# ehsan886/DBA_mod

Hardware: AMD Instinct MI355X
Metric: FL rounds/sec + backdoor ASR & main-task acc, ResNet-18 CIFAR-10 100 clients (higher is better)
Workload: dtype fp32

## Files before the change

### csrc/kernels/xaux.hip

```cpp
#include "common.hpp"
#include "xmfma.hpp"
#include <algorithm>

namespace {

__device__ __forceinline__ void xsplit_w_body(const float* __restrict__ w, long long sstride, long long per,
                                              const int* __restrict__ amax, int ld, uint16_t* __restrict__ out,
                                              int sl, long long e0, long long e1, long long step) {
  const int sb = hexp(amax_read(amax, ld, sl));
  const float mb = __uint_as_float((uint32_t)(sb + 127) << 23);
  const float* __restrict__ src = w + (long long)sl * sstride;
  uint16_t* __restrict__ oh = out + (long long)sl * 2 * per;
  uint16_t* __restrict__ ol = oh + per;
  for (long long e = e0 + threadIdx.x * 4LL; e < e1; e += step) {
    float v[4];
#pragma unroll
    for (int i = 0; i < 4; ++i) v[i] = e + i < per ? src[e + i] : 0.f;
    uint2 sp[2];
    split4h(v[0], v[1], v[2], v[3], mb, sp);
    const uint16_t* h = (const uint16_t*)&sp[0];
    const uint16_t* l = (const uint16_t*)&sp[1];
#pragma unroll
    for (int i = 0; i < 4; ++i)
      if (e + i < per) { oh[e + i] = h[i]; ol[e + i] = l[i]; }
  }
}
__global__ __launch_bounds__(256) void xsplit_w_kernel(const float* __restrict__ w, long long sstride, long long per,
                                                       const int* __restrict__ amax, int ld,
                                                       uint16_t* __restrict__ out) {
  xsplit_w_body(w, sstride, per, amax, ld, out, blockIdx.y, blockIdx.x * 1024LL, per, (long long)gridDim.x * 1024);
}
struct XSDesc {
  long long w, sstride, per, amax, ld, out, boff;
};
constexpr int kXSBatch = 24, kXSChunk = 4096;
struct XSBatch {
  XSDesc d[kXSBatch];
  int n;
};
__global__ __launch_bounds__(256) void xsplit_w_batch_kernel(const XSBatch b) {
  int i = 0;
  while (i + 1 < b.n && (long long)blockIdx.x >= b.d[i + 1].boff) ++i;
  const XSDesc& d = b.d[i];
  const long long e0 = ((long long)blockIdx.x - d.boff) * kXSChunk;
  const long long e1 = e0 + kXSChunk < d.per ? e0 + kXSChunk : d.per;
  xsplit_w_body((const float*)d.w, d.sstride, d.per, (const int*)d.amax, (int)d.ld, (uint16_t*)d.out, blockIdx.y, e0,
                e1, 1024);
}

constexpr int kAmaxSegs = 64, kAmaxChunk = 4096;
struct AmaxSegs {
  long long off[kAmaxSegs];
  int len[kAmaxSegs];
  int start[kAmaxSegs + 1];
  int n;
};
__global__ __launch_bounds__(256) void amax_segments_kernel(const float* __restrict__ base, long long gstride,
                                                            const AmaxSegs segs, int ld, int* __restrict__ out) {
  const int c = blockIdx.x, g = blockIdx.y;
  int sg = 0;
  while (sg + 1 < segs.n && segs.start[sg + 1] <= c) ++sg;
  const float* __restrict__ p = base + (long long)g * gstride + segs.off[sg];
  const int n = segs.len[sg], e0 = (c - segs.start[sg]) * kAmaxChunk;
  const bool v4 = ((segs.off[sg] | gstride) & 3) == 0 && ((uintptr_t)base & 15) == 0;
  float m = 0.f;
  float4 v[4];
#pragma unroll
  for (int k = 0; k < 4; ++k) {
    const int e = e0 + (k * 256 + threadIdx.x) * 4;
    if (v4 && e + 3 < n) {
      v[k] = *(const float4*)(p + e);
    } else {
      v[k].x = e < n ? p[e] : 0.f;
      v[k].y = e + 1 < n ? p[e + 1] : 0.f;
      v[k].z = e + 2 < n ? p[e + 2] : 0.f;
      v[k].w = e + 3 < n ? p[e + 3] : 0.f;
    }
  }
#pragma unroll
  for (int k = 0; k < 4; ++k) m = fmaxf(m, fmaxf(fmaxf(fabsf(v[k].x), fabsf(v[k].y)), fmaxf(fabsf(v[k].z), fabsf(v[k].w))));
  amax_fold(out + (long long)sg * kAmaxSub * ld, ld, g, m);
}

__global__ __launch_bounds__(256) void amax_kernel(const float* __restrict__ x, long long gstride, long long n_per_g,
                                                   const int* __restrict__ nvalid, long long per_item, int vec,
                                                   int* __restrict__ out, int ld) {
  const int g = blockIdx.y;
  const long long n = nvalid ? (long long)nvalid[g] * per_item : n_per_g;
  const float* __restrict__ p = x + (long long)g * gstride;
  float m = 0.f;
  if (vec) {
    const long long n4 = n >> 2;
    for (long long e = blockIdx.x * 256LL + threadIdx.x; e < n4; e += (long long)gridDim.x * 256) {
      const float4 v = ((const float4*)p)[e];
      m = fmaxf(m, fmaxf(fmaxf(fabsf(v.x), fabsf(v.y)), fmaxf(fabsf(v.z), fabsf(v.w))));
    }
    for (long long e = n4 * 4 + blockIdx.x * 256LL + threadIdx.x; e < n; e += (long long)gridDim.x * 256)
      m = fmaxf(m, fabsf(p[e]));
  } else {
    for (long long e = blockIdx.x * 256LL + threadIdx.x; e < n; e += (long long)gridDim.x * 256) m = fmaxf(m, fabsf(p[e]));
  }
  amax_fold(out, ld, g, m);
}

}

DBA_EXPORT int dba_xsplit_w(const float* w, long long sstride, long long per, int slots, const int* amax, int ld,
                            uint16_t* out, void* stream) {
  const dim3 grid((unsigned)std::max(1LL, std::min(1024LL, (per + 1023) / 1024)), slots);
  hipLaunchKernelGGL(xsplit_w_kernel, grid, dim3(256), 0, (hipStream_t)stream, w, sstride, per, amax, ld, out);
  DBA_LAUNCH_CHECK();
}


DBA_EXPORT int dba_xsplit_w_batch(const void* desc, int n, int slots, void* stream) {
  const XSDesc* ds = (const XSDesc*)desc;
  for (int i0 = 0; i0 < n; i0 += kXSBatch) {
    XSBatch b{};
    b.n = std::min(kXSBatch, n - i0);
    long long nb = 0;
    for (int i = 0; i < b.n; ++i) {
      b.d[i] = ds[i0 + i];
      b.d[i].boff = nb;
      nb += (b.d[i].per + kXSChunk - 1) / kXSChunk;
    }
    hipLaunchKernelGGL(xsplit_w_batch_kernel, dim3((unsigned)nb, slots), dim3(256), 0, (hipStream_t)stream, b);
    const int rc = (int)hipGetLastError();
    if (rc != 0) return rc;
  }
  return 0;
}


DBA_EXPORT int dba_amax_segments(const float* base, long long gstride, const long long* segs, int n, int G, int* out,
                                 int ld, void* stream) {
  if (n > kAmaxSegs || n < 1) return -105;
  AmaxSegs a{};
  a.n = n;
  for (int i = 0; i < n; ++i) {
    a.off[i] = segs[2 * i];
    a.len[i] = (int)segs[2 * i + 1];
    a.start[i + 1] = a.start[i] + std::max(1, ceil_div(a.len[i], kAmaxChunk));
  }
  const dim3 grid((unsigned)a.start[n], G);
  hipLaunchKernelGGL(amax_segments_kernel, grid, dim3(256), 0, (hipStream_t)stream, base, gstride, a, ld, out);
  DBA_LAUNCH_CHECK();
}


DBA_EXPORT int dba_amax(const float* x, long long gstride, long long n_per_g, const int* nvalid, long long per_item,
                        int G, int* out, int ld, void* stream) {
  hipStream_t st = (hipStream_t)stream;
  const int vec = aligned16(x) && gstride % 4 == 0;
  const long long per = nvalid ? per_item * (n_per_g / std::max(1LL, per_item)) : n_per_g;
  const dim3 grid((unsigned)std::max(1LL, std::min(256LL, (per + 4095) / 4096)), G);
  hipLaunchKernelGGL(amax_kernel, grid, dim3(256), 0, st, x, gstride, n_per_g, nvalid, per_item, vec, out, ld);
  DBA_LAUNCH_CHECK();
}
```

### csrc/kernels/xconv.hpp

```cpp
#pragma once
#include "common.hpp"
#include "bnfuse.hpp"
#include "xmfma.hpp"
#include <algorithm>
#include <type_traits>
#include <utility>
#include <cstdlib>

namespace xg {
struct SplitPolicy {
  int target = 128, min_k = 8, max_s = 8, kslab_max = 2;
  int dgrad_ks = 1;
};
SplitPolicy& split_policy();
int bnx_tile_go(const ::BnFuse& f, const float* src, float* dst, long long gstride, const int* nvalid, int G, int N,
                int HW, const float* pool, float pool_scale, const float* ws, int S, long long zstride,
                const float* accum, hipStream_t st);
}
using xg::SplitPolicy;
using xg::split_policy;
using xg::bnx_tile_go;

namespace {

struct XClass {
  int nI, nJ;
  int bh, bw;
  int oh, ow;
  int Hq, Wq;
  long long boff;
};

struct XArgs {
  const float* src; long long src_gstride;
  const float* w; long long w_sstride;
  const int* wsel;
  const float* bias; long long b_sstride;
  const float* res;
  float* out; long long out_gstride;
  const int* nvalid;
  int N, Hs, Ws, Cs, Ncol, Ho, Wo;
  int sp, os, dsg, relu;
  int splitk, tiles_n;
  int kslab;
  long long zstride;
  const int* amax_src;
  const int* amax_w;
  int* amax_out;
  int amax_src_ld, amax_w_ld, amax_out_ld;
  const uint16_t* wp;
  long long wp_sstride;
  float* sk_ws; long long sk_gstride;
  int* sk_cnt;
  BnFuse bf;
  const float* lz_coef;
  int lz_relu;
  const float* sc_src; long long sc_gstride;
  int sc_H, sc_W, sc_C;
  const uint16_t* sc_wp; long long sc_wp_sstride;
  const int* sc_amax_src; int sc_amax_src_ld;
  const int* sc_amax_w; int sc_amax_w_ld;
  const float* sc_bias; long long sc_b_sstride;
  XClass cls[4];
};

typedef __attribute__((ext_vector_type(4))) unsigned int u32x4v;

constexpr int kSkMax = 8;
template <int BM, int BN>
__device__ __forceinline__ bool sk_combine(const XArgs& a, float* Ct, const long long* orow, int g, int zc, int kz,
                                           int n0, int* flag) {
  constexpr int C4 = BN / 4, IT = BM * C4 / 256;
  static_assert(BM * C4 % 256 == 0, "whole float4 passes");
  const int tid = threadIdx.x, S = a.splitk;
  const float* base = a.sk_ws + (long long)g * a.sk_gstride;
  int off[IT];
#pragma unroll
  for (int it = 0; it < IT; ++it) {
    const int e = tid + it * 256, row = e / C4, cc = (e - row * C4) * 4, n = n0 + cc;
    const long long o = orow[row];
    off[it] = (o < 0 || n >= a.Ncol) ? kOOB : (int)((o + n) * 4);
  }
  {
    const __amdgpu_buffer_rsrc_t rs = rsrc(base + (long long)kz * a.zstride, a.sk_gstride * 4);
#pragma unroll
    for (int it = 0; it < IT; ++it) {
      const int e = tid + it * 256, row = e / C4, cc = (e - row * C4) * 4;
      const float4 v = *(const float4*)&Ct[row * BN + cc];
      if (off[it] != kOOB)
        __builtin_amdgcn_raw_buffer_store_b128(__builtin_bit_cast(u32x4v, v), rs, off[it], 0, 16);
    }
  }
  asm volatile("s_waitcnt vmcnt(0)" ::: "memory");
  __syncthreads();
  if (tid == 0) {
    int* cnt = a.sk_cnt + ((long long)g * gridDim.x + blockIdx.x) * (gridDim.z / S) + zc;
    const int t = __hip_atomic_fetch_add(cnt, 1, __ATOMIC_RELAXED, __HIP_MEMORY_SCOPE_AGENT);
    const int last = t == S - 1;
    if (last) __hip_atomic_store(cnt, 0, __ATOMIC_RELAXED, __HIP_MEMORY_SCOPE_AGENT);
    *flag = last;
  }
  __syncthreads();
  if (!*flag) return false;
  __builtin_amdgcn_fence(__ATOMIC_ACQUIRE, "wavefront");
  float4 w[kSkMax][IT];
#pragma unroll
  for (int z = 0; z < kSkMax; ++z) {
    if (z < S && z != kz) {
      const __amdgpu_buffer_rsrc_t rz = rsrc(base + (long long)z * a.zstride, a.sk_gstride * 4);
#pragma unroll
      for (int it = 0; it < IT; ++it)
        w[z][it] = __builtin_bit_cast(float4, __builtin_amdgcn_raw_buffer_load_b128(rz, off[it], 0, 16));
    }
  }
#pragma unroll
  for (int it = 0; it < IT; ++it) {
    const int e = tid + it * 256, row = e / C4, cc = (e - row * C4) * 4;
    float4* cp = (float4*)&Ct[row * BN + cc];
    const float4 own = *cp;
    float4 v = kz == 0 ? own : w[0][it];
#pragma unroll
    for (int z = 1; z < kSkMax; ++z) {
      if (z < S) {
        const float4 u = z == kz ? own : w[z][it];
        v.x += u.x; v.y += u.y; v.z += u.z; v.w += u.w;
      }
    }
    if (off[it] != kOOB) *cp = v;
  }
  __syncthreads();
  return true;
}

#ifndef XCONV_MINB
// ... 437 lines not shown
```

### csrc/kernels/xconv_fwd.hip

```cpp
#include "xhalo.hpp"

namespace xg {
SplitPolicy& split_policy() {
  static SplitPolicy p;
  return p;
}
}

namespace {

template <int W, int IMGS, int BN, int WM, int WN, bool PRE>
__global__ __launch_bounds__(256) void ximg_kernel(const XArgs a) {
  constexpr int P = 2, NT = 256;
  constexpr int PW = W + 2, PI = PW * PW, PP = IMGS * PI;
  constexpr int CC = 32, CH = CC / 8, Q4 = CC / 4;
  constexpr int PATCH = PP * CH;
  constexpr int BM = IMGS * W * W;
  constexpr int TM = BM / WM, TN = BN / WN, MI = TM / 32, NJ = TN / 32;
  static_assert(WM * WN == NT / 64 && MI >= 1 && NJ >= 1 && BM == 128, "tiling");
  constexpr int RPT = NT / 8;
  static_assert(BN % RPT == 0, "weight rows");
  constexpr int RB = BN / RPT, BPL = BN * 4;
  __shared__ __attribute__((aligned(16))) uint4 patch[P * PATCH];
  __shared__ __attribute__((aligned(16))) uint4 bring[2 * P * BPL];
// ... 98 lines not shown
#pragma unroll
      for (int i = 0; i < MI; ++i) {
        const int pp = apix[i] + toff;
        const int o = pp * CH + (ch ^ ((arow[i] + ti) & 3));
#pragma unroll
        for (int p = 0; p < P; ++p) af[p][i] = patch[p * PATCH + o];
      }
#pragma unroll
      for (int j = 0; j < NJ; ++j) {
        const int n = wn * TN + j * 32 + fr;
        const int o = n * 4 + (ch ^ ((n >> 2) & 3));
#pragma unroll
        for (int p = 0; p < P; ++p) bfr[p][j] = L[p * BPL + o];
      }
      mma_half<MI, NJ, P, true, RB, decltype(KK)::value>(af, bfr, acc, [&](int q) __attribute__((always_inline)) {
        lput_q(buf ^ 1, stn, q);
        gq(t + 3, stn, q);
      });
    });
  };
  auto step = [&](int t, int buf, int stn) __attribute__((always_inline)) {
    const int c = t / 9;
    mma(t, buf, stn);
    __syncthreads();
    if (t - 9 * c == 8 && c + 1 < NC) {
#pragma unroll
      for (int u = 0; u < NE; ++u) ppiece(u, hs.ma);
      if (c + 2 < NC) pload(c + 2);
      __syncthreads();
    }
  };

  hs.init(amax_read(a.amax_src, a.amax_src_ld, g), amax_read(a.amax_w, a.amax_w_ld, slot));
#pragma unroll
  for (int q = 0; q < RB; ++q) {
    gq(0, 0, q);
    gq(1, 1, q);
  }
  pload(0);
#pragma unroll
  for (int u = 0; u < NE; ++u) ppiece(u, hs.ma);
  if (NC > 1) pload(1);
#pragma unroll
  for (int q = 0; q < RB; ++q) {
    lput_q(0, 0, q);
    gq(2, 0, q);
  }
  __syncthreads();
  int t = 0;
  for (; t + 1 < NK; t += 2) {
    step(t, 0, 1);
    step(t + 1, 1, 0);
  }
  if (t < NK) step(t, 0, 1);
  hs.finish(acc);

  float* out = a.out + (long long)g * a.out_gstride;
  const float* bias = a.bias ? a.bias + (long long)slot * a.b_sstride : nullptr;
  const float* res = a.res ? a.res + (long long)g * a.out_gstride : nullptr;
  float vmax = 0.f;
#pragma unroll
  for (int j = 0; j < NJ; ++j) {
    const int n = n0 + wn * TN + j * 32 + fr;
    if (n >= a.Ncol) continue;
    const float bv = bias ? bias[n] : 0.f;
#pragma unroll
    for (int i = 0; i < MI; ++i)
#pragma unroll
      for (int r = 0; r < 16; ++r) {
        const int m = wm * TM + i * 32 + (r & 3) + 8 * (r >> 2) + 4 * hf;
        if (img0 + m / (W * W) >= nv) continue;
        const long long o = (long long)(img0 * W * W + m) * a.Ncol + n;
        float v = acc[i][j][r];
        if (bias) v += bv;
        if (res) v += res[o];
        if (a.relu) v = fmaxf(v, 0.f);
        vmax = fmaxf(vmax, fabsf(v));
        out[o] = v;
      }
  }
  if (a.amax_out) amax_fold(a.amax_out, a.amax_out_ld, g, vmax);
}

template <int W, int IMGS, int BN, int WM, int WN>
int ximg_go(const XArgs& a, int G, hipStream_t st) {
  XArgs b = a;
  b.tiles_n = ceil_div(a.Ncol, BN);
  const dim3 grid((unsigned)(ceil_div(a.N, IMGS) * b.tiles_n), G, 1);
  if (a.wp) hipLaunchKernelGGL((ximg_kernel<W, IMGS, BN, WM, WN, true>), grid, dim3(256), 0, st, b);
  else hipLaunchKernelGGL((ximg_kernel<W, IMGS, BN, WM, WN, false>), grid, dim3(256), 0, st, b);
  DBA_LAUNCH_CHECK();
}
int& ximg_on() {
  static int on = 1;
  return on;
}
int ximg_try(const XArgs& a, int G, int KH, int KW, hipStream_t st) {
  const XClass& c = a.cls[0];
  if (!ximg_on() || KH != 3 || KW != 3 || a.sp != 1 || a.os != 1 || a.dsg != 1 || a.splitk != 1 || c.nI != 3 ||
      c.nJ != 3 || c.bh != -1 || c.bw != -1)
    return -100;
  if (a.Hs != a.Ho || a.Ws != a.Wo || a.Ho != a.Wo || a.Cs % 32 != 0 || a.Ncol % 32 != 0) return -100;
  if (a.bf.mode || a.lz_coef) return -100;
  if (!aligned16(a.src) || a.src_gstride % 4 || !aligned16(a.w) || a.w_sstride % 4) return -100;
  if (a.wp && (((uintptr_t)a.wp & 15) || a.wp_sstride % 8)) return -100;
  if (a.sc_src) return -100;
  if (a.Wo == 8) return a.Ncol >= 128 ? ximg_go<8, 2, 128, 2, 2>(a, G, st) : ximg_go<8, 2, 64, 2, 2>(a, G, st);
  if (a.Wo == 4) return a.Ncol >= 128 ? ximg_go<4, 8, 128, 2, 2>(a, G, st) : ximg_go<4, 8, 64, 2, 2>(a, G, st);
  return -100;
}

}

DBA_EXPORT int dba_xsplit_policy(int target, int min_k, int max_s, int kslab_max, int dgrad_ks) {
  SplitPolicy& p = split_policy();
  if (dgrad_ks >= 0) p.dgrad_ks = dgrad_ks;
  if (target > 0) p.target = target;
  if (min_k > 0) p.min_k = min_k;
  if (max_s > 0) p.max_s = std::min(max_s, kSkMax);
  if (kslab_max > 0) p.kslab_max = kslab_max;
  return 0;
}

DBA_EXPORT int dba_ximg_set(int on) {
  const int prev = ximg_on();
  if (on >= 0) ximg_on() = on;
  return prev;
}


DBA_EXPORT long long dba_xconv_ws_floats(int G, int N, int Ho, int Wo, int Cin, int Cout, int KH, int KW) {
  const long long M = (long long)N * Ho * Wo;
  const int s = xsplitk(M, G, Cout, KH * KW * Cin);
  return s > 1 ? (long long)s * G * M * Cout : 0;
}


DBA_EXPORT long long dba_xconv_sk_ints(int G, int N, int Ho, int Wo, int Cin, int Cout, int KH, int KW) {
  const long long M = (long long)N * Ho * Wo;
  const int s = xsplitk(M, G, Cout, KH * KW * Cin);
  const long long n = s > 1 ? xconv_sk_count(M, Cout, G, 1, s) : 0;
  return (n > 0 && sk_ok((const int*)1, n, M, Cout, G, 1, s)) ? n : 0;
}


DBA_EXPORT int dba_xconv_fwd(const float* x, long long x_gstride, const float* w, long long w_sstride,
                             const int* wsel, const float* bias, long long b_sstride, const float* res, float* out,
                             long long out_gstride, const int* nvalid, int G, int N, int H, int W, int Cin, int Ho,
                             int Wo, int Cout, int KH, int KW, int stride, int pad, int relu, const int* amax_x,
                             int amax_x_ld, const int* amax_w, int amax_w_ld, int* amax_out, int amax_out_ld,
                             const uint16_t* wp, long long wp_sstride, float* ws, long long ws_floats, int* sk_cnt,
                             long long sk_cnt_n, const void* bnf, const float* lz_coef, int lz_relu,
                             void* stream) {
  hipStream_t st = (hipStream_t)stream;
  if ((long long)N * H * W * Cin >= (1LL << 29)) return -103;
  const long long M = (long long)N * Ho * Wo;
  const int K = KH * KW * Cin;
  const int vec = (Cin % 4 == 0 && aligned16(x) && aligned16(w) && x_gstride % 4 == 0 && w_sstride % 4 == 0) ? 4 : 1;
  XArgs a{};
  a.src = x; a.src_gstride = x_gstride; a.w = w; a.w_sstride = w_sstride; a.wsel = wsel;
  a.bias = bias; a.b_sstride = b_sstride; a.res = res; a.out = out; a.out_gstride = out_gstride;
  a.nvalid = nvalid; a.N = N; a.Hs = H; a.Ws = W; a.Cs = Cin; a.Ncol = Cout; a.Ho = Ho; a.Wo = Wo;
  a.sp = stride; a.os = 1; a.dsg = 1; a.relu = relu; a.splitk = 1;
  a.amax_src = amax_x; a.amax_w = amax_w; a.amax_out = amax_out;
  a.amax_src_ld = amax_x_ld; a.amax_w_ld = amax_w_ld; a.amax_out_ld = amax_out_ld;
  a.wp = wp; a.wp_sstride = wp_sstride;
  a.cls[0] = XClass{KH, KW, -pad, -pad, 0, 0, Ho, Wo, 0};
  if (!amax_x || !amax_w) return -109;
  if (bnf) {
    a.bf = *(const BnFuse*)bnf;
    if (a.bf.mode != 1 || bias || res || relu || (Cout & 3) || a.bf.C != Cout) return -108;
  }
  if (lz_coef) {
    if (wp || vec < 4 || Cin > 512) return -108;
    a.lz_coef = lz_coef; a.lz_relu = lz_relu;
  }
  auto fin = [&](int rc) { return (rc == 0 && a.bf.mode) ? bnx_finalize_go(a.bf, nvalid, G, N, Ho * Wo, st) : rc; };
  if (stride == 1) {
    int rc = ximg_try(a, G, KH, KW, st);
    if (rc == -100) rc = xhalo_try(a, G, KH, KW, st);
    if (rc != -100) return fin(rc);
  }
  const int s = xsplitk(M, G, Cout, K);
  const bool ws_ok = s > 1 && ws != nullptr && ws_floats >= (long long)s * G * M * Cout;
  if (s > 1 && !(ws_ok && sk_ok(sk_cnt, sk_cnt_n, M, Cout, G, 1, s))) {
    XArgs b = a;
    b.kslab = s;
    const int rc = xconv_ks(b, M, G, vec, st);
    if (rc != -100) return fin(rc);
  }
  if (ws_ok && sk_ok(sk_cnt, sk_cnt_n, M, Cout, G, 1, s)) {
    XArgs b = a;
    b.splitk = s;
    b.zstride = (long long)G * M * Cout;
    b.sk_ws = ws; b.sk_gstride = M * Cout; b.sk_cnt = sk_cnt;
    return fin(xconv_dispatch(b, M, G, 1, vec, st));
  }
  if (ws_ok) {
    XArgs b = a;
    b.splitk = s;
    b.out = ws;
    b.out_gstride = M * Cout;
    b.zstride = (long long)G * M * Cout;
    const int rc = xconv_dispatch(b, M, G, 1, vec, st);
    if (rc != 0) return rc;
    if (a.bf.mode)
      return bnx_tile_go(a.bf, nullptr, out, out_gstride, nvalid, G, N, Ho * Wo, nullptr, 0.f, ws, s, b.zstride,
                         nullptr, st);
    const long long per = M * Cout;
    const dim3 grid((unsigned)std::max(1LL, std::min(1024LL, (per + 255) / 256)), G);
    hipLaunchKernelGGL(xsplitk_reduce_kernel, grid, dim3(256), 0, st, (const float*)ws, s, b.zstride, per, nvalid, N,
                       Ho * Wo, Cout, bias, b_sstride, wsel, res, relu, out, amax_out, amax_out_ld);
    DBA_LAUNCH_CHECK();
  }
  return fin(xconv_dispatch(a, M, G, 1, vec, st));
}


DBA_EXPORT int dba_xdown_fwd(const float* a_, long long a_gstride, const float* w2, long long w2_sstride,
                             const uint16_t* w2p, long long w2p_sstride, const int* wsel, const float* b2,
                             long long b_sstride, const float* x2, long long x2_gstride, const uint16_t* wscp,
                             long long wscp_sstride, const float* bsc, long long bsc_sstride, float* out,
                             long long out_gstride, const int* nvalid, int G, int N, int Ho, int Wo, int C, int H2,
                             int W2, int C2, const int* amax_a, int amax_a_ld, const int* amax_w2, int amax_w2_ld,
                             const int* amax_x2, int amax_x2_ld, const int* amax_wsc, int amax_wsc_ld, int* amax_out,
                             int amax_out_ld, void* stream) {
  if (!amax_a || !amax_w2 || !amax_x2 || !amax_wsc || !w2p || !wscp) return -109;
  if ((H2 - 1) / 2 + 1 != Ho || (W2 - 1) / 2 + 1 != Wo || (long long)N * H2 * W2 * C2 >= (1LL << 29) ||
      (long long)N * Ho * Wo * C >= (1LL << 29))
    return -103;
  XArgs a{};
  a.src = a_; a.src_gstride = a_gstride; a.w = w2; a.w_sstride = w2_sstride; a.wsel = wsel;
  a.bias = b2; a.b_sstride = b_sstride; a.res = nullptr; a.out = out; a.out_gstride = out_gstride;
  a.nvalid = nvalid; a.N = N; a.Hs = Ho; a.Ws = Wo; a.Cs = C; a.Ncol = C; a.Ho = Ho; a.Wo = Wo;
  a.sp = 1; a.os = 1; a.dsg = 1; a.relu = 1; a.splitk = 1;
  a.amax_src = amax_a; a.amax_w = amax_w2; a.amax_out = amax_out;
  a.amax_src_ld = amax_a_ld; a.amax_w_ld = amax_w2_ld; a.amax_out_ld = amax_out_ld;
  a.wp = w2p; a.wp_sstride = w2p_sstride;
  a.sc_src = x2; a.sc_gstride = x2_gstride; a.sc_H = H2; a.sc_W = W2; a.sc_C = C2;
  a.sc_wp = wscp; a.sc_wp_sstride = wscp_sstride;
  a.sc_amax_src = amax_x2; a.sc_amax_src_ld = amax_x2_ld; a.sc_amax_w = amax_wsc; a.sc_amax_w_ld = amax_wsc_ld;
  a.sc_bias = bsc; a.sc_b_sstride = bsc_sstride;
  a.cls[0] = XClass{3, 3, -1, -1, 0, 0, Ho, Wo, 0};
  return xhalo_try(a, G, 3, 3, (hipStream_t)stream);
}
```

### dba_mod_amd/ops/hip.py

```python
from __future__ import annotations

import contextlib
import ctypes
import os
from typing import Optional, Sequence, Tuple

import torch

from . import bnstate as bs
from . import build

Tensor = torch.Tensor
_F32 = torch.float32

if not os.path.exists(build.kernels_path()):
    raise ImportError(f"HIP kernel library missing: {build.kernels_path()} — run "
                      f"`python -m dba_mod_amd.ops.build` (or __graft_entry__.build())")
_L = ctypes.CDLL(build.kernels_path())

_P = ctypes.c_void_p
_I = ctypes.c_int
_LL = ctypes.c_longlong
_F = ctypes.c_float
_U = ctypes.c_uint
_D = ctypes.c_double

_SIGS = {
    "dba_gather_images": [_P, _P, _P, _P, _P, _P, _I, _P, _P, _I, _P, _I, _I, _I, _I, _I, _P],
    "dba_gather_rows": [_P, _P, _P, _P, _P, _I, _P, _P, _I, _P, _I, _P, _I, _I, _I, _P],
    "dba_xcolsum": [_P, _LL, _I, _P, _I, _I, _I, _P, _LL, _P, _P],
    "dba_xcolsum_part_doubles": [_I, _I, _I, _I],
    "dba_amax_segments": [_P, _LL, _P, _I, _I, _P, _I, _P],
    "dba_bn_fold": [_P, _LL, _P, _P, _P, _P, _P, _LL, _F, _P, _P, _I, _I, _I, _I, _P, _I, _P],
    "dba_relu_mask_bwd": [_P, _P, _P, _LL, _I, _P],
    "dba_maxpool": [_P, _P, _P, _LL, _I, _I, _I, _I, _I, _I, _I, _I, _I, _P],
    "dba_maxpool_bwd": [_P, _P, _P, _LL, _I, _I, _I, _I, _I, _I, _I, _I, _I, _P],
    "dba_avgpool": [_P, _P, _LL, _I, _I, _I, _P],
    "dba_avgpool_bwd": [_P, _P, _LL, _I, _I, _I, _P],
    "dba_dropout": [_P, _P, _I, _P, _U, _F, _LL, _I, _P],
    "dba_softmax_xent": [_P, _P, _I, _I, _I, _I, _P, _P, _P, _P, _LL, _P, _I, _P, _I, _P, _P, _P],
    "dba_softmax_xent_part_doubles": [_I, _I],
    "dba_xent_r5_set": [_I],
    "dba_head_train": [_P, _LL, _I, _I, _I, _I, _P, _LL, _P, _LL, _I, _P, _P, _P, _P, _P, _P, _LL, _P, _LL, _P, _P,
                       _P, _P, _LL, _P, _I, _I, _P],
    "dba_head_part_doubles": [_I, _I],
    "dba_sgd_step": [_P, _LL, _P, _P, _P, _P, _P, _F, _F, _P, _I, _I, _P],
    "dba_scale_from_base": [_P, _P, _F, _P, _LL, _P],
    "dba_add_noise_scaled": [_P, _P, _LL, _F, _F, _U, _I, _I, _P],
    "dba_delta_sum": [_P, _LL, _I, _P, _LL, _P, _P],
    "dba_sqdist_blocks": [_LL],
    "dba_gram_chunks": [_I],
    "dba_sq_dists": [_P, _LL, _P, _I, _LL, _P, _P, _P],
    "dba_weighted_sum": [_P, _LL, _P, _I, _P, _LL, _I, _P],
    "dba_weighted_sum_fixed": [_P, _LL, _P, _I, _P, _LL, _D, _P],
    "dba_gram": [_P, _LL, _I, _I, _P, _P, _P],
    "dba_dist_loss_grad": [_P, _LL, _P, _LL, _P, _LL, _I, _P, _P, _F, _P, _P, _P],
    "dba_ximg_set": [_I],
    "dba_xwgrad_halo_set": [_I],
    "dba_xconv_ws_floats": [_I] * 8,
    "dba_xconv_fwd": [_P, _LL, _P, _LL, _P, _P, _LL, _P, _P, _LL, _P] + [_I] * 13 + [_P, _I] * 3 + [_P, _LL] * 2
    + [_P, _LL, _P, _P, _I, _P],
    "dba_xconv_sk_ints": [_I] * 8,
    "dba_xconv_dgrad": [_P, _LL, _P, _LL, _P, _P, _P, _LL, _P] + [_I] * 12 + [_P, _I] * 2 + [_P, _LL] * 3 + [_P, _P],
    "dba_xsplit_w": [_P, _LL, _LL, _I, _P, _I, _P, _P],
    "dba_amax": [_P, _LL, _LL, _P, _LL, _I, _P, _I, _P],
    "dba_xtranspose": [_P, _I, _I, _LL, _P, _P],
    "dba_xwgrad_ws_floats": [_I] * 8 + [_P],
    "dba_xwgrad_stem_ws_floats": [_I] * 6,
    "dba_xsplit_policy": [_I] * 5,
    "dba_xsplit_w_batch": [_P, _I, _I, _P],
    "dba_bn_fold_batch": [_P, _I, _I, _F, _P],
    "dba_xwgrad": [_P, _LL, _P, _LL, _P, _LL, _P] + [_I] * 12 + [_P, _I] * 2 + [_P, _LL, _I] + [_P, _I, _P],
    "dba_bnx_rows": [_P, _P, _P, _LL, _P, _I, _I, _I, _P, _F, _P],
    "dba_bnx_apply": [_P, _P, _P, _P, _P, _I, _I, _P, _LL, _P, _I, _I, _I, _I, _P, _I, _P],
    "dba_bnfuse_size": [],
    "dba_xwgrad_stem": [_P, _LL, _P, _P, _P, _LL, _P, _P, _I, _I, _I, _I, _P],
    "dba_bnx_dy": [_P, _P, _P, _P, _LL, _P, _I, _I, _I, _I, _P, _I, _P],
    "dba_xwgrad_reduce_batch": [_P, _I, _I, _LL, _P],
    "dba_xblock_fwd": [_P, _LL, _P, _LL, _P, _P, _P, _LL, _P, _P, _LL, _P] + [_I] * 6
    + [_P, _I, _P, _P, _I, _P, _I, _P],
    "dba_xblock_stem_fwd": [_P, _LL, _P, _LL, _P, _P, _LL, _P, _LL, _P, _P, _LL, _P, _P, _LL, _P] + [_I] * 6
    + [_P, _P, _P, _I, _P, _I, _P],
    "dba_mlp_train": [_P, _I, _I, _I, _I, _I, _P, _LL, _P, _P, _I, _P, _I, _I, _I, _I, _P, _P, _P, _P, _I, _I,
                      _P, _LL, _I, _P, _F, _F, _P, _P],
    "dba_xdown_fwd": [_P, _LL, _P, _LL, _P, _LL, _P, _P, _LL, _P, _LL, _P, _LL, _P, _LL, _P, _LL, _P] + [_I] * 8
    + [_P, _I] * 5 + [_P],
    "dba_xstem_fwd": [_P, _LL, _P, _LL, _P, _P, _LL, _P, _P, _LL, _P] + [_I] * 13 + [_P, _I, _P, _P],
}
for _name, _args in _SIGS.items():
    _fn = getattr(_L, _name)
    _fn.argtypes = _args
    _fn.restype = ctypes.c_int
_L.dba_xconv_ws_floats.restype = ctypes.c_longlong
_L.dba_xconv_sk_ints.restype = ctypes.c_longlong
_L.dba_xwgrad_ws_floats.restype = ctypes.c_longlong
_L.dba_xwgrad_stem_ws_floats.restype = ctypes.c_longlong
_L.dba_xcolsum_part_doubles.restype = ctypes.c_longlong
_L.dba_softmax_xent_part_doubles.restype = ctypes.c_longlong
_L.dba_head_part_doubles.restype = ctypes.c_longlong


class _BnFuse(ctypes.Structure):
    _fields_ = [("mode", _I), ("C", _I), ("ngrp", _I),
                ("rec0", _P),
                ("coef_a", _P), ("gamma_a", _P), ("beta_a", _P), ("rm_a", _P), ("rv_a", _P),
                ("p_gstride", _LL), ("momentum", _F), ("eps", _F), ("relu", _I),
                ("amax_a", _P), ("amax_ld", _I),
                ("ya", _P), ("yb", _P), ("y_gstride", _LL),
                ("coef_b", _P), ("gamma_b", _P), ("amax_b", _P),
                ("dgamma_a", _P), ("dbeta_a", _P), ("dgamma_b", _P), ("dbeta_b", _P), ("gr_gstride", _LL),
                ("mask_out", _P), ("mask_lazy", _I)]


assert ctypes.sizeof(_BnFuse) == int(_L.dba_bnfuse_size()), "BnFuse layout mismatch (rebuild the kernels)"


NOT_HANDLED = -100
F16_PAIR = 16


def _call(name: str, *args) -> int:
    rc = getattr(_L, name)(*args)
    if rc != 0 and rc != NOT_HANDLED:
        raise RuntimeError(f"{name}: HIP error {rc}")
    return rc


def _ptr(t: Optional[Tensor]):
    return None if t is None else t.data_ptr()


def _stream():
    return torch.cuda.current_stream().cuda_stream


def _i32(t: Optional[Tensor]) -> Optional[Tensor]:
    if t is None:
        return None
    return t if (t.dtype == torch.int32 and t.is_contiguous()) else t.to(torch.int32).contiguous()


def _inner_contig(t: Tensor) -> bool:
    exp = 1
    for d in range(t.dim() - 1, 0, -1):
        if t.shape[d] != 1 and t.stride(d) != exp:
            return False
        exp *= t.shape[d]
    return True


def _rowview(t: Tensor) -> Tuple[Tensor, int]:
    if not _inner_contig(t):
        t = t.contiguous()
# ... 121 lines not shown
        flat = torch.zeros(slots + counters, dtype=torch.int32, device=device)
        self.buf = flat[:slots].view(n, AMAX_SUB, self.ld)
        self.cnt, self.cnt_next = flat[slots:], 0

    def counters(self, n: int, device):
        if n <= 0 or device != self.cnt.device or self.cnt_next + n > self.cnt.numel():
            return None
        self.cnt_next += n
        return self.cnt[self.cnt_next - n:self.cnt_next]

    def take(self, G: int, device):
        if G != self.G or self.next >= self.buf.shape[0] or device != self.buf.device:
            return None
        self.next += 1
        return self.buf[self.next - 1]


_ARENA: list = []


@contextlib.contextmanager
def amax_arena(G: int, device, n: int = 256, counters: int = 0):
    _ARENA.append(_AmaxArena(G, device, n, counters))
    try:
        yield
    finally:
        _ARENA.pop()


def amax_slots(n: int, G: int, device):
    return torch.zeros(n, AMAX_SUB, _amax_ld(G), dtype=torch.int32, device=device)


def _amax_new(G: int, device):
    a = _ARENA[-1].take(G, device) if _ARENA else None
    return a if a is not None else torch.zeros(AMAX_SUB, _amax_ld(G), dtype=torch.int32, device=device)


def _sk_counters(n: int, device):
    if n <= 0 or not _ARENA:
        return None
    return _ARENA[-1].counters(n, device)


def _aptr(a):
    return (None, 0) if a is None else (a.data_ptr(), a.shape[-1])


def _amax(t, gstride, n_per_g, nvalid=None, per_item=0):
    G = t.shape[0]
    out = _amax_new(G, t.device)
    _call("dba_amax", t.data_ptr(), gstride, n_per_g, _ptr(_i32(nvalid)), per_item, G, out.data_ptr(), out.shape[1],
          _stream())
    return out


def _amax_out(t):
    if t.dtype != _F32:
        return None
    a = _amax_new(t.shape[0], t.device)
    t._dba_amax = a
    return a


def weight_amax(flat, segments):
    G, n = flat.shape[0], len(segments)
    ar = _ARENA[-1] if _ARENA else None
    if ar is not None and ar.G == G and ar.buf.device == flat.device and ar.next + n <= ar.buf.shape[0]:
        buf, ar.next = ar.buf[ar.next:ar.next + n], ar.next + n
    else:
        buf = torch.zeros(n, AMAX_SUB, _amax_ld(G), dtype=torch.int32, device=flat.device)
    slots, base = list(buf), buf.data_ptr()
    d = torch.tensor(segments, dtype=torch.int64)
    _call("dba_amax_segments", flat.data_ptr(), flat.stride(0), d.data_ptr(), len(segments), G, base,
          slots[0].shape[1], _stream())
    return slots


def split_weights(w, sstride: int, per: int, amax):
    slots = w.shape[0]
    out = torch.empty(slots, 2, per, dtype=torch.int16, device=w.device)
    _call("dba_xsplit_w", w.data_ptr(), sstride, per, slots, amax.data_ptr(), amax.shape[1], out.data_ptr(), _stream())
    w._dba_planes = out
    return out


def split_weights_batch(items) -> None:
    if not items:
        return
    slots = items[0][0].shape[0]
    desc, outs = [], []
    for w, sstride, per, amax in items:
        assert w.shape[0] == slots and w.dtype == torch.float32
        out = torch.empty(slots, 2, per, dtype=torch.int16, device=w.device)
        desc.append([w.data_ptr(), sstride, per, amax.data_ptr(), amax.shape[1], out.data_ptr(), 0])
        outs.append(out)
    d = torch.tensor(desc, dtype=torch.int64)
    _call("dba_xsplit_w_batch", d.data_ptr(), len(items), slots, _stream())
    for (w, *_), out in zip(items, outs):
        w._dba_planes = out


def _wplanes(w):
    p = getattr(w, "_dba_planes", None)
    return (None, 0) if p is None else (p.data_ptr(), p.stride(0))


def _amax_w(w, gstride, n):
    a = getattr(w, "_dba_amax", None)
    if a is None:
        a = _amax(w, gstride, n)
        w._dba_amax = a
    return a


def _amax_act(t, nvalid):
    a = getattr(t, "_dba_amax", None)
    if a is not None:
        return a
    per_item = t[0, 0].numel()
    a = _amax(t, t.stride(0), t.shape[1] * per_item, nvalid, per_item)
    t._dba_amax = a
    return a


_EVAL_STEM_MFMA = os.environ.get("DBA_EVAL_STEM7_MFMA", "1") != "0"
_EVAL_STEM_PAD = True


def _xconv_fwd(x, w, wsel, stride, pad, bias, residual, relu, nvalid, out_dtype, bnf=None, lz=None):
    if out_dtype not in (None, _F32):
        raise TypeError(f"fp32 conv cannot emit {out_dtype} (no silent precision conversion)")
    G, N, H, W, Cin = x.shape
    attrs = {k: getattr(w, k) for k in ("_dba_amax", "_dba_planes") if hasattr(w, k)}
    w, ws = _check_w(w, _F32)
    for k, v in attrs.items():
        setattr(w, k, v)
    Cout, KH, KW = w.shape[1], w.shape[2], w.shape[3]
    assert w.shape[4] == Cin, (w.shape, x.shape)
    Ho = (H + 2 * pad - KH) // stride + 1
    Wo = (W + 2 * pad - KW) // stride + 1
    y = torch.empty(G, N, Ho, Wo, Cout, dtype=_F32, device=x.device)
    bs = 0
    if bias is not None:
        if bias.dtype != _F32:
            raise TypeError(f"conv bias must be fp32 (got {bias.dtype})")
        bias, bs = _rowview(bias)
    res = _act(residual, _F32, "residual") if residual is not None else None
    ay = _amax_out(y) if bnf is None else None
    bnf_p = ctypes.byref(bnf) if bnf is not None else None
    eval_mfma = (_EVAL_STEM_MFMA and "_dba_planes" in attrs and bnf is None and KH * KW * Cin > 64)
    if eval_mfma and Cin % 4 and _EVAL_STEM_PAD and lz is None:
        cp = 4 - Cin % 4
        x4 = torch.nn.functional.pad(x, (0, cp))
        x4._dba_amax = _amax_act(x, nvalid)
        w4 = torch.nn.functional.pad(w, (0, cp)).contiguous()
        per4 = w4[0].numel()
        a4 = attrs.get("_dba_amax")
        split_weights(w4, per4, per4, a4 if a4 is not None else _amax_w(w4, per4, per4))
        if a4 is not None:
            w4._dba_amax = a4
        return _xconv_fwd(x4, w4, wsel, stride, pad, bias, residual, relu, nvalid, out_dtype)
    if Cin <= 4 and not eval_mfma:
        rc = _call("dba_xstem_fwd", x.data_ptr(), N * H * W * Cin, w.data_ptr(), ws, _ptr(_i32(wsel)), _ptr(bias), bs,
                   _ptr(res), y.data_ptr(), N * Ho * Wo * Cout, _ptr(_i32(nvalid)), G, N, H, W, Cin, Ho, Wo, Cout,
                   KH, KW, stride, pad, int(relu), *_aptr(ay), bnf_p, _stream())
        if rc != NOT_HANDLED:
            return y
    n = int(_L.dba_xconv_ws_floats(G, N, Ho, Wo, Cin, Cout, KH, KW))
    wsb = torch.empty(n, dtype=_F32, device=x.device) if n > 0 else None
    ncnt = int(_L.dba_xconv_sk_ints(G, N, Ho, Wo, Cin, Cout, KH, KW)) if n > 0 else 0
    cnt = _sk_counters(ncnt, x.device)
    ax = lz[2] if lz is not None else _amax_act(x, nvalid)
    aw = _amax_w(w, ws, Cout * KH * KW * Cin)
    lz_coef, lz_relu = (lz[0].data_ptr(), int(lz[1])) if lz is not None else (None, 0)
    _call("dba_xconv_fwd", x.data_ptr(), N * H * W * Cin, w.data_ptr(), ws, _ptr(_i32(wsel)), _ptr(bias), bs,
          _ptr(res), y.data_ptr(), N * Ho * Wo * Cout, _ptr(_i32(nvalid)), G, N, H, W, Cin, Ho, Wo, Cout, KH, KW,
          stride, pad, int(relu), *_aptr(ax), *_aptr(aw), *_aptr(ay), *_wplanes(w), _ptr(wsb), n,
          _ptr(cnt), 0 if cnt is None else cnt.numel(), bnf_p, lz_coef, lz_relu, _stream())
    return y


_EVAL_BLOCK = os.environ.get("DBA_EVAL_BLOCK", "1") != "0"
_BLOCK_SHAPES = {(32, 32)}


def basic_block_ok(x, w1, w2) -> bool:
    if not (_EVAL_BLOCK and x.dtype == _F32 and x.dim() == 5):
        return False
    H, W, C = x.shape[2:]
    return (H == W and (W, C) in _BLOCK_SHAPES
            and all(w.dtype == _F32 and tuple(w.shape[1:]) == (C, 3, 3, C)
                    and getattr(w, "_dba_planes", None) is not None for w in (w1, w2)))


def basic_block_eval(x, w1, b1, w2, b2, wsel=None, nvalid=None):
    x = _act(x, _F32, "conv input")
    G, N, _, W, C = x.shape
    per = C * 9 * C
    (w1c, ws1), (w2c, ws2) = _check_w(w1), _check_w(w2)
    aw1, aw2 = _amax_w(w1, ws1, per), _amax_w(w2, ws2, per)
    p1, p2 = w1._dba_planes, w2._dba_planes
    assert p1.stride(0) == p2.stride(0) and aw1.shape[1] == aw2.shape[1]
    (b1c, bs1), (b2c, bs2) = _rowview(b1), _rowview(b2)
    assert bs1 == bs2 and b1c.dtype == b2c.dtype == _F32
    ax = _amax_act(x, nvalid)
    y = torch.empty_like(x)
    ay = _amax_out(y)
    rc = _call("dba_xblock_fwd", x.data_ptr(), x.stride(0), y.data_ptr(), y.stride(0), _ptr(_i32(wsel)),
               p1.data_ptr(), p2.data_ptr(), p1.stride(0), b1c.data_ptr(), b2c.data_ptr(), bs1, _ptr(_i32(nvalid)),
               G, N, W, W, C, C, *_aptr(ax), aw1.data_ptr(), aw2.data_ptr(), aw1.shape[1], *_aptr(ay), _stream())
    if rc == NOT_HANDLED:
        raise RuntimeError("xblock_fwd declined a shape basic_block_ok accepted")
    return y


_EVAL_STEM = os.environ.get("DBA_EVAL_STEM", "1") != "0"


def stem_block_ok(x, w0, w1, w2) -> bool:
    if not (_EVAL_STEM and _EVAL_BLOCK and x.dtype == _F32 and x.dim() == 5 and tuple(x.shape[2:]) == (32, 32, 3)):
        return False
    return (w0.dtype == _F32 and tuple(w0.shape[1:]) == (32, 3, 3, 3) and getattr(w0, "_dba_planes", None) is not None
            and all(w.dtype == _F32 and tuple(w.shape[1:]) == (32, 3, 3, 32)
                    and getattr(w, "_dba_planes", None) is not None for w in (w1, w2)))


def stem_block_eval(x, w0, b0, w1, b1, w2, b2, wsel=None, nvalid=None):
    x = _act(x, _F32, "image")
    G, N, _, W, Ci = x.shape
    C = w1.shape[1]
    per = C * 9 * C
    (w0c, ws0), (w1c, ws1), (w2c, ws2) = _check_w(w0), _check_w(w1), _check_w(w2)
    aw0 = _amax_w(w0, ws0, C * 9 * Ci)
    aw1, aw2 = _amax_w(w1, ws1, per), _amax_w(w2, ws2, per)
    p0, p1, p2 = w0._dba_planes, w1._dba_planes, w2._dba_planes
    assert p1.stride(0) == p2.stride(0) and aw0.shape[1] == aw1.shape[1] == aw2.shape[1]
    (b0c, bs0), (b1c, bs1), (b2c, bs2) = _rowview(b0), _rowview(b1), _rowview(b2)
    assert bs1 == bs2 and b0c.dtype == b1c.dtype == b2c.dtype == _F32
    y = torch.empty(G, N, W, W, C, dtype=_F32, device=x.device)
    ay = _amax_out(y)
    rc = _call("dba_xblock_stem_fwd", x.data_ptr(), x.stride(0), y.data_ptr(), y.stride(0), _ptr(_i32(wsel)),
               p0.data_ptr(), p0.stride(0), b0c.data_ptr(), bs0, p1.data_ptr(), p2.data_ptr(), p1.stride(0),
               b1c.data_ptr(), b2c.data_ptr(), bs1, _ptr(_i32(nvalid)), G, N, W, W, Ci, C, aw0.data_ptr(),
               aw1.data_ptr(), aw2.data_ptr(), aw1.shape[1], *_aptr(ay), _stream())
    if rc == NOT_HANDLED:
        raise RuntimeError("xblock_stem_fwd declined a shape stem_block_ok accepted")
    return y


def down_block_ok(a, w2, x2, wsc) -> bool:
    if not (_EVAL_DOWN and a.dtype == _F32 and x2.dtype == _F32 and a.dim() == 5 and x2.dim() == 5):
        return False
    H, W, C = a.shape[2:]
    H2, W2, C2 = x2.shape[2:]
    if H != W or (H2 - 1) // 2 + 1 != H or (W2 - 1) // 2 + 1 != W or a.shape[:2] != x2.shape[:2]:
        return False
    if any(getattr(t, "_dba_planes", None) is None for t in (w2, wsc)):
        return False
    if tuple(w2.shape[1:]) != (C, 3, 3, C) or tuple(wsc.shape[1:]) != (C, 1, 1, C2):
        return False
# ... 572 lines not shown
```

Baseline: 3.627.

## Add pre-fragmented weight planes and LDS-patch img conv kernel for small spatial layers

Adds a batched kernel that rearranges the split hi/lo bf16 weight planes into an MFMA fragment-ordered layout, so each lane can fetch its B fragment with one 16-byte load. It also adds a new ximg2 forward kernel for 8x8 and 4x4 outputs that stages a padded, swizzled input patch in double-buffered LDS and pipelines weight-fragment loads across the nine taps. The aim is to cut global weight gathers and per-tap address work. In exchange it runs an extra rearrangement pass and keeps an extra weight copy in memory each time weights are split.

```diff
diff --git a/csrc/kernels/xaux.hip b/csrc/kernels/xaux.hip
--- a/csrc/kernels/xaux.hip
+++ b/csrc/kernels/xaux.hip
@@ -46,6 +46,30 @@
   const long long e1 = e0 + kXSChunk < d.per ? e0 + kXSChunk : d.per;
   xsplit_w_body((const float*)d.w, d.sstride, d.per, (const int*)d.amax, (int)d.ld, (uint16_t*)d.out, blockIdx.y, e0,
                 e1, 1024);
+}
+
+struct XFDesc {
+  long long planes, out, ncol, cs, boff;
+};
+struct XFBatch {
+  XFDesc d[kXSBatch];
+  int n;
+};
+__global__ __launch_bounds__(256) void xfrag_w_kernel(const XFBatch b) {
+  int i = 0;
+  while (i + 1 < b.n && (long long)blockIdx.x >= b.d[i + 1].boff) ++i;
+  const XFDesc& d = b.d[i];
+  const int Cs = (int)d.cs, K = 9 * Cs, NK = K / 32;
+  const long long per = d.ncol * K;
+  const long long idx = ((long long)blockIdx.x - d.boff) * 256 + threadIdx.x;
+  if (idx >= per / 4) return;
+  const int l = (int)(idx & 63), f = (int)(idx >> 6) & 3, p = f & 1, kk = f >> 1;
+  const long long tt = idx >> 8;
+  const int t = (int)(tt % NK), nt = (int)(tt / NK), cc = t / 9, tap = t - cc * 9;
+  const long long e = (long long)(nt * 32 + (l & 31)) * K + tap * Cs + cc * 32 + (kk * 2 + (l >> 5)) * 8;
+  const uint16_t* __restrict__ src = (const uint16_t*)d.planes + ((long long)blockIdx.y * 2 + p) * per;
+  uint16_t* __restrict__ dst = (uint16_t*)d.out + (long long)blockIdx.y * 2 * per;
+  ((uint4*)dst)[idx] = *(const uint4*)(src + e);
 }
 
 constexpr int kAmaxSegs = 64, kAmaxChunk = 4096;
@@ -132,6 +156,27 @@
 }
 
 
+DBA_EXPORT int dba_xfrag_w_batch(const void* desc, int n, int slots, void* stream) {
+  const XFDesc* ds = (const XFDesc*)desc;
+  for (int i0 = 0; i0 < n; i0 += kXSBatch) {
+    XFBatch b{};
+    b.n = std::min(kXSBatch, n - i0);
+    long long nb = 0;
+    for (int i = 0; i < b.n; ++i) {
+      b.d[i] = ds[i0 + i];
+      if (b.d[i].ncol <= 0 || b.d[i].cs <= 0 || b.d[i].ncol % 32 || b.d[i].cs % 32 || ((b.d[i].planes | b.d[i].out) & 15))
+        return -105;
+      b.d[i].boff = nb;
+      nb += b.d[i].ncol * 9 * b.d[i].cs / 1024;
+    }
+    hipLaunchKernelGGL(xfrag_w_kernel, dim3((unsigned)nb, slots), dim3(256), 0, (hipStream_t)stream, b);
+    const int rc = (int)hipGetLastError();
+    if (rc != 0) return rc;
+  }
+  return 0;
+}
+
+
 DBA_EXPORT int dba_amax_segments(const float* base, long long gstride, const long long* segs, int n, int G, int* out,
                                  int ld, void* stream) {
   if (n > kAmaxSegs || n < 1) return -105;
diff --git a/csrc/kernels/xconv.hpp b/csrc/kernels/xconv.hpp
--- a/csrc/kernels/xconv.hpp
+++ b/csrc/kernels/xconv.hpp
@@ -50,6 +50,8 @@
   int amax_src_ld, amax_w_ld, amax_out_ld;
   const uint16_t* wp;
   long long wp_sstride;
+  const uint16_t* wf;
+  long long wf_sstride;
   float* sk_ws; long long sk_gstride;
   int* sk_cnt;
   BnFuse bf;
diff --git a/csrc/kernels/xconv_fwd.hip b/csrc/kernels/xconv_fwd.hip
--- a/csrc/kernels/xconv_fwd.hip
+++ b/csrc/kernels/xconv_fwd.hip
@@ -204,6 +204,151 @@
   if (a.amax_out) amax_fold(a.amax_out, a.amax_out_ld, g, vmax);
 }
 
+template <int W, int IMGS, int BN>
+__global__ __launch_bounds__(256) void ximg2_kernel(const XArgs a) {
+  constexpr int P = 2, NT = 256;
+  constexpr int PW = W + 2, PI = PW * PW, PP = IMGS * PI;
+  constexpr int CC = 32, CH = CC / 8, Q4 = CC / 4;
+  constexpr int PATCH = PP * CH;
+  constexpr int BM = IMGS * W * W;
+  constexpr int WN = BN / 32, WM = (NT / 64) / WN, TM = BM / WM, MI = TM / 32;
+  static_assert(WM * WN == NT / 64 && MI >= 1 && BM == 128, "tiling");
+  extern __shared__ __attribute__((aligned(16))) uint4 ximg2_patch[];
+
+  const int g = blockIdx.y;
+  const int tn = blockIdx.x % a.tiles_n, tm = blockIdx.x / a.tiles_n;
+  const int img0 = tm * IMGS, n0 = tn * BN;
+  const int nv = min(valid_rows(a.nvalid, g, a.N), a.N);
+  if (img0 >= nv) return;
+  const int slot = a.wsel ? a.wsel[g] : g;
+  const int Cs = a.Cs, NC = Cs / CC, NK = 9 * NC;
+  const float* __restrict__ src = a.src + (long long)g * a.src_gstride;
+  const int tid = threadIdx.x, lane = tid & 63, wid = tid >> 6;
+  const int wm = wid / WN, wn = wid % WN;
+  const int fr = lane & 31, hf = lane >> 5;
+
+  constexpr int NE = (PP * Q4 + NT - 1) / NT;
+  static_assert(NE <= 9, "one patch piece per k-step");
+  float4 pv[NE];
+  const __amdgpu_buffer_rsrc_t rA = rsrc(src, (long long)a.N * W * W * Cs * 4);
+  auto pload1 = [&](int u, int cc) __attribute__((always_inline)) {
+    const int e = tid + NT * u;
+    const int pp = e / Q4, q = e - pp * Q4;
+    const int im = pp / PI, rem = pp - im * PI;
+    const int h = rem / PW - 1, w = rem % PW - 1, img = img0 + im;
+    const bool ok = e < PP * Q4 && cc < NC && img < nv && (unsigned)h < (unsigned)W && (unsigned)w < (unsigned)W;
+    pv[u] = bload4(rA, ok ? (((img * W + h) * W + w) * Cs + cc * CC + q * 4) * 4 : kOOB);
+  };
+  HScale hs;
+  auto ppiece = [&](int u, int buf) __attribute__((always_inline)) {
+    const int e = tid + NT * u;
+    if (NT * (u + 1) > PP * Q4 && e >= PP * Q4) return;
+    const int pp = e / Q4, q = e - pp * Q4;
+    const int prow = (pp % PI) / PW;
+    uint2 sp[P];
+    split4h(pv[u].x, pv[u].y, pv[u].z, pv[u].w, hs.ma, sp);
+    const int o = pp * CH + ((q >> 1) ^ (prow & 3));
+#pragma unroll
+    for (int p = 0; p < P; ++p) ((uint2*)&ximg2_patch[(buf * P + p) * PATCH + o])[q & 1] = sp[p];
+  };
+
+  const __amdgpu_buffer_rsrc_t rF = rsrc(a.wf + (long long)slot * a.wf_sstride, (long long)a.Ncol * 9 * Cs * 4);
+  const int wbase = ((n0 >> 5) + wn) * NK * 4096 + lane * 16;
+  uint4 wb[3][4];
+  auto gw = [&](int t, int s, int f) __attribute__((always_inline)) {
+    wb[s][f] = __builtin_bit_cast(uint4, bload4(rF, t < NK ? wbase + t * 4096 + f * 1024 : kOOB));
+  };
+
+  f32x16_t acc[MI][1];
+#pragma unroll
+  for (int i = 0; i < MI; ++i)
+#pragma unroll
+    for (int r = 0; r < 16; ++r) acc[i][0][r] = 0.f;
+
+  int apix[MI], arow[MI];
+#pragma unroll
+  for (int i = 0; i < MI; ++i) {
+    const int m = wm * TM + i * 32 + fr;
+    const int im = m / (W * W), rem = m - im * (W * W);
+    apix[i] = im * PI + (rem / W) * PW + rem % W;
+    arow[i] = rem / W;
+  }
+
+  hs.init(amax_read(a.amax_src, a.amax_src_ld, g), amax_read(a.amax_w, a.amax_w_ld, slot));
+#pragma unroll
+  for (int f = 0; f < 4; ++f) {
+    gw(0, 0, f);
+    gw(1, 1, f);
+  }
+#pragma unroll
+  for (int u = 0; u < NE; ++u) pload1(u, 0);
+#pragma unroll
+  for (int u = 0; u < NE; ++u) {
+    ppiece(u, 0);
+    pload1(u, 1);
+  }
+  __syncthreads();
+  for (int c = 0; c < NC; ++c) {
+    const uint4* L = ximg2_patch + (c & 1) * P * PATCH;
+    const bool more = c + 1 < NC;
+    sfor<9>([&](auto TAP) __attribute__((always_inline)) {
+      constexpr int tap = decltype(TAP)::value, ti = tap / 3, tj = tap - ti * 3;
+      constexpr int toff = ti * PW + tj, s = tap % 3, s2 = (tap + 2) % 3;
+      constexpr int u = tap - (9 - NE);
+      constexpr int NQ = u >= 0 ? 5 : 4;
+      const int t = c * 9 + tap;
+      __builtin_amdgcn_sched_barrier(0x786);
+      sfor<2>([&](auto KK) __attribute__((always_inline)) {
+        constexpr int kk = decltype(KK)::value;
+        const int ch = kk * 2 + hf;
+        uint4 af[P][MI], bfr[P][1];
+#pragma unroll
+        for (int i = 0; i < MI; ++i) {
+          const int o = (apix[i] + toff) * CH + (ch ^ ((arow[i] + ti) & 3));
+#pragma unroll
+          for (int p = 0; p < P; ++p) af[p][i] = L[p * PATCH + o];
+        }
+#pragma unroll
+        for (int p = 0; p < P; ++p) bfr[p][0] = wb[s][kk * 2 + p];
+        mma_half<MI, 1, P, true, NQ, kk>(af, bfr, acc, [&](int q) __attribute__((always_inline)) {
+          if (q < 4) {
+            gw(t + 2, s2, q);
+          } else if constexpr (u >= 0) {
+            if (more) ppiece(u, (c + 1) & 1);
+            pload1(u, c + 2);
+          }
+        });
+      });
+    });
+    __syncthreads();
+  }
+  hs.finish(acc);
+
+  float* out = a.out + (long long)g * a.out_gstride;
+  const float* bias = a.bias ? a.bias + (long long)slot * a.b_sstride : nullptr;
+  const float* res = a.res ? a.res + (long long)g * a.out_gstride : nullptr;
+  float vmax = 0.f;
+  const int n = n0 + wn * 32 + fr;
+  if (n < a.Ncol) {
+    const float bv = bias ? bias[n] : 0.f;
+#pragma unroll
+    for (int i = 0; i < MI; ++i)
+#pragma unroll
+      for (int r = 0; r < 16; ++r) {
+        const int m = wm * TM + i * 32 + (r & 3) + 8 * (r >> 2) + 4 * hf;
+        if (img0 + m / (W * W) >= nv) continue;
+        const long long o = (long long)(img0 * W * W + m) * a.Ncol + n;
+        float v = acc[i][0][r];
+        if (bias) v += bv;
+        if (res) v += res[o];
+        if (a.relu) v = fmaxf(v, 0.f);
+        vmax = fmaxf(vmax, fabsf(v));
+        out[o] = v;
+      }
+  }
+  if (a.amax_out) amax_fold(a.amax_out, a.amax_out_ld, g, vmax);
+}
+
 template <int W, int IMGS, int BN, int WM, int WN>
 int ximg_go(const XArgs& a, int G, hipStream_t st) {
   XArgs b = a;
@@ -211,6 +356,25 @@
   const dim3 grid((unsigned)(ceil_div(a.N, IMGS) * b.tiles_n), G, 1);
   if (a.wp) hipLaunchKernelGGL((ximg_kernel<W, IMGS, BN, WM, WN, true>), grid, dim3(256), 0, st, b);
   else hipLaunchKernelGGL((ximg_kernel<W, IMGS, BN, WM, WN, false>), grid, dim3(256), 0, st, b);
+  DBA_LAUNCH_CHECK();
+}
+template <int W, int IMGS, int BN>
+int ximg2_go(const XArgs& a, int G, hipStream_t st) {
+  constexpr int PATCH = IMGS * (W + 2) * (W + 2) * 4;
+  constexpr int LDS = 2 * 2 * PATCH * (int)sizeof(uint4);
+  static unsigned long long attr_set = 0ull;
+  int dev = 0;
+  if (hipGetDevice(&dev) != hipSuccess || dev < 0 || dev >= 64) return -100;
+  if (!(attr_set >> dev & 1ull)) {
+    if (hipFuncSetAttribute((const void*)ximg2_kernel<W, IMGS, BN>, hipFuncAttributeMaxDynamicSharedMemorySize,
+                            LDS) != hipSuccess)
+      return -100;
+    attr_set |= 1ull << dev;
+  }
+  XArgs b = a;
+  b.tiles_n = ceil_div(a.Ncol, BN);
+  const dim3 grid((unsigned)(ceil_div(a.N, IMGS) * b.tiles_n), G, 1);
+  hipLaunchKernelGGL((ximg2_kernel<W, IMGS, BN>), grid, dim3(256), LDS, st, b);
   DBA_LAUNCH_CHECK();
 }
 int& ximg_on() {
@@ -227,6 +391,12 @@
   if (!aligned16(a.src) || a.src_gstride % 4 || !aligned16(a.w) || a.w_sstride % 4) return -100;
   if (a.wp && (((uintptr_t)a.wp & 15) || a.wp_sstride % 8)) return -100;
   if (a.sc_src) return -100;
+  if (ximg_on() == 1 && a.wp && a.wf && !((uintptr_t)a.wf & 15) && a.wf_sstride % 8 == 0) {
+    int rc = -100;
+    if (a.Wo == 8) rc = a.Ncol >= 128 ? ximg2_go<8, 2, 128>(a, G, st) : ximg2_go<8, 2, 64>(a, G, st);
+    if (a.Wo == 4) rc = a.Ncol >= 128 ? ximg2_go<4, 8, 128>(a, G, st) : ximg2_go<4, 8, 64>(a, G, st);
+    if (rc != -100) return rc;
+  }
   if (a.Wo == 8) return a.Ncol >= 128 ? ximg_go<8, 2, 128, 2, 2>(a, G, st) : ximg_go<8, 2, 64, 2, 2>(a, G, st);
   if (a.Wo == 4) return a.Ncol >= 128 ? ximg_go<4, 8, 128, 2, 2>(a, G, st) : ximg_go<4, 8, 64, 2, 2>(a, G, st);
   return -100;
@@ -271,7 +441,8 @@
                              long long out_gstride, const int* nvalid, int G, int N, int H, int W, int Cin, int Ho,
                              int Wo, int Cout, int KH, int KW, int stride, int pad, int relu, const int* amax_x,
                              int amax_x_ld, const int* amax_w, int amax_w_ld, int* amax_out, int amax_out_ld,
-                             const uint16_t* wp, long long wp_sstride, float* ws, long long ws_floats, int* sk_cnt,
+                             const uint16_t* wp, long long wp_sstride, const uint16_t* wf, long long wf_sstride,
+                             float* ws, long long ws_floats, int* sk_cnt,
                              long long sk_cnt_n, const void* bnf, const float* lz_coef, int lz_relu,
                              void* stream) {
   hipStream_t st = (hipStream_t)stream;
@@ -286,7 +457,7 @@
   a.sp = stride; a.os = 1; a.dsg = 1; a.relu = relu; a.splitk = 1;
   a.amax_src = amax_x; a.amax_w = amax_w; a.amax_out = amax_out;
   a.amax_src_ld = amax_x_ld; a.amax_w_ld = amax_w_ld; a.amax_out_ld = amax_out_ld;
-  a.wp = wp; a.wp_sstride = wp_sstride;
+  a.wp = wp; a.wp_sstride = wp_sstride; a.wf = wf; a.wf_sstride = wf_sstride;
   a.cls[0] = XClass{KH, KW, -pad, -pad, 0, 0, Ho, Wo, 0};
   if (!amax_x || !amax_w) return -109;
   if (bnf) {
diff --git a/dba_mod_amd/ops/hip.py b/dba_mod_amd/ops/hip.py
--- a/dba_mod_amd/ops/hip.py
+++ b/dba_mod_amd/ops/hip.py
@@ -58,7 +58,7 @@
     "dba_ximg_set": [_I],
     "dba_xwgrad_halo_set": [_I],
     "dba_xconv_ws_floats": [_I] * 8,
-    "dba_xconv_fwd": [_P, _LL, _P, _LL, _P, _P, _LL, _P, _P, _LL, _P] + [_I] * 13 + [_P, _I] * 3 + [_P, _LL] * 2
+    "dba_xconv_fwd": [_P, _LL, _P, _LL, _P, _P, _LL, _P, _P, _LL, _P] + [_I] * 13 + [_P, _I] * 3 + [_P, _LL] * 3
     + [_P, _LL, _P, _P, _I, _P],
     "dba_xconv_sk_ints": [_I] * 8,
     "dba_xconv_dgrad": [_P, _LL, _P, _LL, _P, _P, _P, _LL, _P] + [_I] * 12 + [_P, _I] * 2 + [_P, _LL] * 3 + [_P, _P],
@@ -69,6 +69,7 @@
     "dba_xwgrad_stem_ws_floats": [_I] * 6,
     "dba_xsplit_policy": [_I] * 5,
     "dba_xsplit_w_batch": [_P, _I, _I, _P],
+    "dba_xfrag_w_batch": [_P, _I, _I, _P],
     "dba_bn_fold_batch": [_P, _I, _I, _F, _P],
     "dba_xwgrad": [_P, _LL, _P, _LL, _P, _LL, _P] + [_I] * 12 + [_P, _I] * 2 + [_P, _LL, _I] + [_P, _I, _P],
     "dba_bnx_rows": [_P, _P, _P, _LL, _P, _I, _I, _I, _P, _F, _P],
@@ -356,6 +357,7 @@
     out = torch.empty(slots, 2, per, dtype=torch.int16, device=w.device)
     _call("dba_xsplit_w", w.data_ptr(), sstride, per, slots, amax.data_ptr(), amax.shape[1], out.data_ptr(), _stream())
     w._dba_planes = out
+    frag_weights_batch([w])
     return out
 
 
@@ -373,10 +375,34 @@
     _call("dba_xsplit_w_batch", d.data_ptr(), len(items), slots, _stream())
     for (w, *_), out in zip(items, outs):
         w._dba_planes = out
+    frag_weights_batch([w for w, *_ in items])
+
+
+def frag_weights_batch(ws) -> None:
+    desc, outs = [], []
+    for w in ws:
+        p = getattr(w, "_dba_planes", None)
+        if (p is None or w.dim() != 5 or tuple(w.shape[2:4]) != (3, 3) or w.shape[1] % 32 or w.shape[4] % 32
+                or not p.is_contiguous() or p.shape[2] != w[0].numel()):
+            continue
+        out = torch.empty(p.shape[0], 2 * p.shape[2], dtype=torch.int16, device=p.device)
+        desc.append([p.data_ptr(), out.data_ptr(), w.shape[1], w.shape[4], 0])
+        outs.append((w, out))
+    if not desc:
+        return
+    d = torch.tensor(desc, dtype=torch.int64)
+    _call("dba_xfrag_w_batch", d.data_ptr(), len(desc), outs[0][1].shape[0], _stream())
+    for w, out in outs:
+        w._dba_fplanes = out
 
 
 def _wplanes(w):
     p = getattr(w, "_dba_planes", None)
+    return (None, 0) if p is None else (p.data_ptr(), p.stride(0))
+
+
+def _wfplanes(w):
+    p = getattr(w, "_dba_fplanes", None)
     return (None, 0) if p is None else (p.data_ptr(), p.stride(0))
 
 
@@ -406,7 +432,7 @@
     if out_dtype not in (None, _F32):
         raise TypeError(f"fp32 conv cannot emit {out_dtype} (no silent precision conversion)")
     G, N, H, W, Cin = x.shape
-    attrs = {k: getattr(w, k) for k in ("_dba_amax", "_dba_planes") if hasattr(w, k)}
+    attrs = {k: getattr(w, k) for k in ("_dba_amax", "_dba_planes", "_dba_fplanes") if hasattr(w, k)}
     w, ws = _check_w(w, _F32)
     for k, v in attrs.items():
         setattr(w, k, v)
@@ -450,7 +476,7 @@
     lz_coef, lz_relu = (lz[0].data_ptr(), int(lz[1])) if lz is not None else (None, 0)
     _call("dba_xconv_fwd", x.data_ptr(), N * H * W * Cin, w.data_ptr(), ws, _ptr(_i32(wsel)), _ptr(bias), bs,
           _ptr(res), y.data_ptr(), N * Ho * Wo * Cout, _ptr(_i32(nvalid)), G, N, H, W, Cin, Ho, Wo, Cout, KH, KW,
-          stride, pad, int(relu), *_aptr(ax), *_aptr(aw), *_aptr(ay), *_wplanes(w), _ptr(wsb), n,
+          stride, pad, int(relu), *_aptr(ax), *_aptr(aw), *_aptr(ay), *_wplanes(w), *_wfplanes(w), _ptr(wsb), n,
           _ptr(cnt), 0 if cnt is None else cnt.numel(), bnf_p, lz_coef, lz_relu, _stream())
     return y
 
```

Result: faster. 3.759, median of 6 (+3.6%).
